# SamsungLabs/Metis

Hardware: AMD Instinct MI355X
Metric: best_plan_iter_time_ms (lower is better)
Workload: dtype bf16; 1 GPU; model=gpt3-2.7b, global_batch=16, seq_len=2048, parallelism=dp1_tp1_pp1, microbatch=16

## Files before the change

metis_amd/ops/hip/attention.hip:

```cpp

#include <torch/extension.h>
#include <c10/hip/HIPStream.h>

#include "attn_host.h"
#include "attn_tile.h"

namespace {

using namespace attn_tile;

constexpr int THREADS = 256;
constexpr int QBLK = 128;
constexpr int RESIDENT = 2;
static_assert(QBLK == ATTN_SEQ_TILE, "check_attn_qkv pins S to this tile");

template <int D>
constexpr int kvblk_for() { return D <= 80 ? 128 : 64; }

template <int D>
using FwdLayout = TileLayout<D, kvblk_for<D>(), THREADS / 64 * 2, RESIDENT>;
static_assert(FwdLayout<64>::bytes == 71680 && FwdLayout<80>::bytes == 79872
              && FwdLayout<96>::bytes == 45056 && FwdLayout<128>::bytes == 53248);

template <int D, bool PACKED>
__global__ __launch_bounds__(THREADS, RESIDENT) void attn_fwd_kernel(
    const bf16* __restrict__ Q,
    const bf16* __restrict__ K,
    const bf16* __restrict__ V,
    bf16* __restrict__ O,
    float* __restrict__ LSE,
    int B, int H, int Hkv, int S,
    float scale) {
    const int lane = threadIdx.x & 63;
    const int wave = threadIdx.x >> 6;
    const int col16 = lane & 15;
    const int k8 = lane >> 4;

    using L = FwdLayout<D>;
    constexpr int KVBLK = kvblk_for<D>();
    constexpr int JSUB = KVBLK / 16;
    constexpr int dchunks = Geom<D>::dchunks;
    constexpr int djtiles = Geom<D>::djtiles;
    constexpr int KSLOT = Geom<D>::KSLOT;
    constexpr int VROW = L::WROW;

    const BlockCoord bc = block_coord<D, PACKED>(S / QBLK, H, Hkv, S);
    const long q_base = bc.q_base;
    const int pitch = bc.qkv_pitch;

    const int rbid[2] = {wave, 7 - wave};
    const int qb = bc.tile * QBLK;

    extern __shared__ __attribute__((aligned(16))) char smem[];
    short* Ks = reinterpret_cast<short*>(smem) + L::a_off;
    short* Vs = reinterpret_cast<short*>(smem) + L::b_off;
    short* Pw = reinterpret_cast<short*>(smem) + L::w_off + wave * 2 * L::w_tile;

    bf16x8 q_frag[2][dchunks];
    #pragma unroll
    for (int rb = 0; rb < 2; ++rb)
        #pragma unroll
        for (int c = 0; c < dchunks; ++c)
            q_frag[rb][c] = frag8<D>(Q + q_base, qb + rbid[rb] * 16 + col16,
                                     c * 32 + k8 * 8, pitch);

    float m_run[2][4], l_run[2][4];
    #pragma unroll
    for (int rb = 0; rb < 2; ++rb)
        #pragma unroll
        for (int r = 0; r < 4; ++r) {
            m_run[rb][r] = -1e30f;
            l_run[rb][r] = 0.f;
        }
    floatx4 o_acc[2][djtiles] = {};

    constexpr Walk WK = PACKED ? Walk::WholeRows : Walk::DChunksInRow;
    constexpr Walk WV = PACKED ? Walk::WholeRows : Walk::RowsInDChunk;
    TileStage<KVBLK, D, THREADS, WK, WV, true,
              PACKED> stage;
    const bf16* Kh = K + bc.kv_base;
    const bf16* Vh = V + bc.kv_base;

    const int kv_end = qb + QBLK;
    stage.issue_loads(Kh, Vh, 0, pitch, pitch);
    for (int kv0 = 0; kv0 < kv_end; kv0 += KVBLK) {
        stage.write_stage(Ks, Vs, Vh, kv0, pitch);
        if (kv0 + KVBLK < kv_end) stage.issue_loads(Kh, Vh, kv0 + KVBLK, pitch,
                                                      pitch);
        __syncthreads();

        bool rb_active[2];
        float p[2][JSUB][4];
        #pragma unroll
        for (int rb = 0; rb < 2; ++rb) {
            const int q0 = qb + rbid[rb] * 16;
            rb_active[rb] = kv0 <= q0 + 15;
            if (!rb_active[rb]) continue;

            __builtin_amdgcn_s_setprio(1);
            #pragma unroll
            for (int j = 0; j < JSUB; ++j) {
                floatx4 s_acc = floatx4{0.f, 0.f, 0.f, 0.f};
                const int kvrow = j * 16 + col16;
                #pragma unroll
                for (int c = 0; c < dchunks; ++c) {
                    const bf16x8 k_frag =
                        lds_frag<D, KSLOT>(Ks, kvrow, c * 32 + k8 * 8);
                    s_acc = __builtin_amdgcn_mfma_f32_16x16x32_bf16(
                        q_frag[rb][c], k_frag, s_acc, 0, 0, 0);
                }
                #pragma unroll
                for (int r = 0; r < 4; ++r) {
                    const int qrow = q0 + k8 * 4 + r;
                    const int kvcol = kv0 + j * 16 + col16;
                    float sv = s_acc[r] * scale;
                    p[rb][j][r] = (kvcol > qrow) ? -1e30f : sv;
                }
            }
            __builtin_amdgcn_s_setprio(0);

            #pragma unroll
            for (int r = 0; r < 4; ++r) {
                float tile_max = -1e30f;
                #pragma unroll
                for (int j = 0; j < JSUB; ++j)
                    tile_max = fmaxf(tile_max, p[rb][j][r]);
                #pragma unroll
                for (int off = 8; off > 0; off >>= 1)
                    tile_max = fmaxf(tile_max, __shfl_xor(tile_max, off, 16));

                const float m_new = fmaxf(m_run[rb][r], tile_max);
                const float alpha = __expf(m_run[rb][r] - m_new);
                float row_sum = 0.f;
                #pragma unroll
                for (int j = 0; j < JSUB; ++j) {
                    p[rb][j][r] = __expf(p[rb][j][r] - m_new);
                    row_sum += p[rb][j][r];
                }
                #pragma unroll
                for (int off = 8; off > 0; off >>= 1)
                    row_sum += __shfl_xor(row_sum, off, 16);

                l_run[rb][r] = l_run[rb][r] * alpha + row_sum;
                m_run[rb][r] = m_new;
                #pragma unroll
                for (int jd = 0; jd < djtiles; ++jd)
                    o_acc[rb][jd][r] *= alpha;
            }

            short* Prb = Pw + rb * 16 * VROW;
            #pragma unroll
            for (int j = 0; j < JSUB; ++j)
                #pragma unroll
                for (int r = 0; r < 4; ++r)
                    Prb[(k8 * 4 + r) * VROW + j * 16 + col16] =
                        float_to_bf16_bits(p[rb][j][r]);
        }

        asm volatile("" ::: "memory");

        #pragma unroll
        for (int rb = 0; rb < 2; ++rb) {
            if (!rb_active[rb]) continue;
            const short* Prb = Pw + rb * 16 * VROW;
            #pragma unroll
            for (int ks = 0; ks < KVBLK / 32; ++ks) {
                bf16x8 p_frag = *reinterpret_cast<const bf16x8*>(
                    Prb + col16 * VROW + ks * 32 + k8 * 8);
                #pragma unroll
                for (int jd = 0; jd < djtiles; ++jd) {
                    const bf16x8 v_frag = tr16_frag<KSLOT>(
                        Vs, ks * 32 + k8 * 8, jd * 16, col16);
                    o_acc[rb][jd] = __builtin_amdgcn_mfma_f32_16x16x32_bf16(
                        p_frag, v_frag, o_acc[rb][jd], 0, 0, 0);
                }
            }
        }
        __syncthreads();
    }

    #pragma unroll
    for (int rb = 0; rb < 2; ++rb) {
        #pragma unroll
        for (int r = 0; r < 4; ++r) {
            const int qrow = qb + rbid[rb] * 16 + k8 * 4 + r;
            const float inv_l = 1.f / l_run[rb][r];
            #pragma unroll
            for (int jd = 0; jd < djtiles; ++jd)
                O[bc.o_base + (long)qrow * bc.o_pitch + jd * 16 + col16] =
                    __float2bfloat16(o_acc[rb][jd][r] * inv_l);
            if (col16 == 0)
                LSE[bc.row_base + qrow] =
                    m_run[rb][r] + __logf(l_run[rb][r]);
        }
    }
}

}

std::vector<torch::Tensor> attn_fwd(
    torch::Tensor q, torch::Tensor k, torch::Tensor v, double scale) {
    const AttnDims a = check_attn_qkv(q, k, v);
    auto qc = q.contiguous(), kc = k.contiguous(), vc = v.contiguous();

    auto o = torch::empty_like(qc);
    auto lse = torch::empty({a.B, a.H, a.S}, q.options().dtype(torch::kFloat32));

    const int grid = (int)(a.B * a.H * (a.S / QBLK));
    auto stream = c10::hip::getCurrentHIPStream().stream();
    dispatch_head_dim(a.D, [&](auto d) {
        constexpr int DD = decltype(d)::value;
        hipLaunchKernelGGL((attn_fwd_kernel<DD, false>), dim3(grid), dim3(THREADS),
            FwdLayout<DD>::bytes, stream,
            bf16_ptr(qc), bf16_ptr(kc), bf16_ptr(vc), bf16_ptr(o),
            lse.data_ptr<float>(),
            (int)a.B, (int)a.H, (int)a.Hkv, (int)a.S, (float)scale);
    });
    HIP_CHECK_LAST();
    return {o, lse};
}

std::vector<torch::Tensor> attn_fwd_packed(
    torch::Tensor qkv, long H, long Hkv, long D, double scale) {
    const AttnDims a = check_attn_packed_qkv(qkv, H, Hkv, D);

    auto o = torch::empty({a.B, a.S, a.H * a.D}, qkv.options());
    auto lse = torch::empty({a.B, a.H, a.S}, qkv.options().dtype(torch::kFloat32));
// ... 16 lines not shown
```

metis_amd/ops/hip/attention_bwd.hip:

```cpp

#include <torch/extension.h>
#include <c10/hip/HIPStream.h>

#include "attn_host.h"
#include "attn_tile.h"

namespace {

using namespace attn_tile;

constexpr int THREADS = 256;
constexpr int RBLK = 128;
constexpr int CTILE = 64;
constexpr int VROW = CTILE + VPAD;
constexpr int RESIDENT = 2;
static_assert(RBLK == ATTN_SEQ_TILE, "check_attn_qkv pins S to this tile");

template <int D>
constexpr int dkv_rows() { return D == 64 ? 128 : 64; }

template <int D>
using DqLayout = TileLayout<D, CTILE, THREADS / 64 * 2, RESIDENT>;
template <int D>
using DkvLayout = TileLayout<D, CTILE, 2 * (dkv_rows<D>() / 16), RESIDENT>;
static_assert(DqLayout<64>::bytes == 36864 && DqLayout<80>::bytes == 40960
              && DqLayout<96>::bytes == 45056 && DqLayout<128>::bytes == 53248);
static_assert(DkvLayout<64>::bytes == 55296 && DkvLayout<80>::bytes == 40960
              && DkvLayout<96>::bytes == 45056 && DkvLayout<128>::bytes == 53248);

template <int D, bool PACKED>
__global__ __launch_bounds__(THREADS, RESIDENT) void attn_bwd_dq_kernel(
    const bf16* __restrict__ Q, const bf16* __restrict__ K,
    const bf16* __restrict__ V, const bf16* __restrict__ dO,
    const float* __restrict__ LSE, const float* __restrict__ Delta,
    bf16* __restrict__ dQ,
    int B, int H, int Hkv, int S, float scale) {
    const int lane = threadIdx.x & 63;
    const int wave = threadIdx.x >> 6;
    const int col16 = lane & 15;
    const int k8 = lane >> 4;

    using L = DqLayout<D>;
    constexpr int dchunks = Geom<D>::dchunks;
    constexpr int djtiles = Geom<D>::djtiles;
    constexpr int KSLOT = Geom<D>::KSLOT;

    const BlockCoord bc = block_coord<D, PACKED>(S / RBLK, H, Hkv, S);
    const long q_base = bc.q_base, row_base = bc.row_base;
    const int pitch = bc.qkv_pitch;

    const int rbid[2] = {wave, 7 - wave};
    const int qb = bc.tile * RBLK;

    extern __shared__ __attribute__((aligned(16))) char smem[];
    short* Ks = reinterpret_cast<short*>(smem) + L::a_off;
    short* Vs = reinterpret_cast<short*>(smem) + L::b_off;
    short* Sw = reinterpret_cast<short*>(smem) + L::w_off + wave * 2 * L::w_tile;

    float lse_r[2][4], delta_r[2][4];
    bf16x8 q_frag[2][dchunks], do_frag[2][dchunks];
    #pragma unroll
    for (int rb = 0; rb < 2; ++rb) {
        const int q0 = qb + rbid[rb] * 16;
        #pragma unroll
        for (int r = 0; r < 4; ++r) {
            lse_r[rb][r] = LSE[row_base + q0 + k8 * 4 + r];
            delta_r[rb][r] = Delta[row_base + q0 + k8 * 4 + r];
        }
        #pragma unroll
        for (int c = 0; c < dchunks; ++c) {
            q_frag[rb][c] = frag8<D>(Q + q_base, q0 + col16, c * 32 + k8 * 8,
                                     pitch);
            do_frag[rb][c] = frag8<D>(dO + bc.o_base, q0 + col16,
                                      c * 32 + k8 * 8, bc.o_pitch);
        }
    }

    floatx4 dq_acc[2][djtiles] = {};

    constexpr Walk WALK = PACKED ? Walk::WholeRows : Walk::RowsInDChunk;
    TileStage<CTILE, D, THREADS, WALK, WALK, false,
              PACKED> stage;
    const bf16* Kh = K + bc.kv_base;
    const bf16* Vh = V + bc.kv_base;

    const int kv_end = qb + RBLK;
    stage.issue_loads(Kh, Vh, 0, pitch, pitch);
    for (int kv0 = 0; kv0 < kv_end; kv0 += CTILE) {
        stage.write_stage(Ks, Vs, Vh, kv0, pitch);
        if (kv0 + CTILE < kv_end)
            stage.issue_loads(Kh, Vh, kv0 + CTILE, pitch, pitch);
        __syncthreads();

        bool rb_active[2];
        #pragma unroll
        for (int rb = 0; rb < 2; ++rb) {
            const int q0 = qb + rbid[rb] * 16;
            rb_active[rb] = kv0 <= q0 + 15;
            if (!rb_active[rb]) continue;

            __builtin_amdgcn_s_setprio(1);
            floatx4 s_acc[4], dp_acc[4];
            #pragma unroll
            for (int j = 0; j < 4; ++j) {
                s_acc[j] = floatx4{0.f, 0.f, 0.f, 0.f};
                dp_acc[j] = floatx4{0.f, 0.f, 0.f, 0.f};
                const int kvrow = j * 16 + col16;
                #pragma unroll
                for (int c = 0; c < dchunks; ++c) {
                    const int d0 = c * 32 + k8 * 8;
                    bf16x8 kf, vf;
                    lds_frag2<D, KSLOT>(Ks, Vs, kvrow, d0, kf, vf);
                    s_acc[j] = __builtin_amdgcn_mfma_f32_16x16x32_bf16(
                        q_frag[rb][c], kf, s_acc[j], 0, 0, 0);
                    dp_acc[j] = __builtin_amdgcn_mfma_f32_16x16x32_bf16(
                        do_frag[rb][c], vf, dp_acc[j], 0, 0, 0);
                }
            }
            __builtin_amdgcn_s_setprio(0);

            short* Srb = Sw + rb * 16 * VROW;
            #pragma unroll
            for (int j = 0; j < 4; ++j)
                #pragma unroll
                for (int r = 0; r < 4; ++r) {
                    const int qrow = q0 + k8 * 4 + r;
                    const int kvcol = kv0 + j * 16 + col16;
                    float p = (kvcol > qrow)
                                  ? 0.f
                                  : __expf(s_acc[j][r] * scale - lse_r[rb][r]);
                    float ds = scale * p * (dp_acc[j][r] - delta_r[rb][r]);
                    Srb[(k8 * 4 + r) * VROW + j * 16 + col16] =
                        float_to_bf16_bits(ds);
                }
        }

        asm volatile("" ::: "memory");

        #pragma unroll
        for (int rb = 0; rb < 2; ++rb) {
            if (!rb_active[rb]) continue;
            const short* Srb = Sw + rb * 16 * VROW;
            #pragma unroll
            for (int ks = 0; ks < 2; ++ks) {
                bf16x8 ds_frag = *reinterpret_cast<const bf16x8*>(
                    Srb + col16 * VROW + ks * 32 + k8 * 8);
                #pragma unroll
                for (int jd = 0; jd < djtiles; ++jd) {
                    bf16x8 kt_frag = tr16_frag<KSLOT>(
                        Ks, ks * 32 + k8 * 8, jd * 16, col16);
                    dq_acc[rb][jd] = __builtin_amdgcn_mfma_f32_16x16x32_bf16(
                        ds_frag, kt_frag, dq_acc[rb][jd], 0, 0, 0);
                }
            }
        }
        __syncthreads();
    }

    #pragma unroll
    for (int rb = 0; rb < 2; ++rb)
        #pragma unroll
        for (int r = 0; r < 4; ++r) {
            const long qrow = qb + rbid[rb] * 16 + k8 * 4 + r;
            #pragma unroll
            for (int jd = 0; jd < djtiles; ++jd)
                dQ[q_base + qrow * pitch + jd * 16 + col16] =
                    __float2bfloat16(dq_acc[rb][jd][r]);
        }
}

template <int D, bool PACKED>
__global__ __launch_bounds__(dkv_rows<D>() / 16 * 64, RESIDENT)
void attn_bwd_dkv_kernel(
    const bf16* __restrict__ Q, const bf16* __restrict__ K,
    const bf16* __restrict__ V, const bf16* __restrict__ dO,
    const float* __restrict__ LSE, const float* __restrict__ Delta,
    bf16* __restrict__ dK,
    bf16* __restrict__ dV,
    int B, int H, int Hkv, int S, float scale) {
    const int lane = threadIdx.x & 63;
    const int wave = threadIdx.x >> 6;
    const int col16 = lane & 15;
    const int k8 = lane >> 4;

    using L = DkvLayout<D>;
    constexpr int dchunks = Geom<D>::dchunks;
    constexpr int djtiles = Geom<D>::djtiles;
    constexpr int KSLOT = Geom<D>::KSLOT;
    constexpr int KVB = dkv_rows<D>();
    constexpr int NW = KVB / 16;

    const BlockCoord bc = block_coord<D, PACKED>(S / KVB, H, Hkv, S);
    const long kv_base = bc.kv_base, row_base = bc.row_base;
    const long out_base = bc.q_base;
    const int pitch = bc.qkv_pitch;

    const int kv0 = bc.tile * KVB + wave * 16;

    extern __shared__ __attribute__((aligned(16))) char smem[];
    short* Qs = reinterpret_cast<short*>(smem) + L::a_off;
    short* dOs = reinterpret_cast<short*>(smem) + L::b_off;
    short* Sw = reinterpret_cast<short*>(smem) + L::w_off + wave * L::w_tile;
    short* Pw = reinterpret_cast<short*>(smem) + L::w_off + (NW + wave) * L::w_tile;

    bf16x8 k_frag[dchunks], v_frag[dchunks];
    #pragma unroll
    for (int c = 0; c < dchunks; ++c) {
        k_frag[c] = frag8<D>(K + kv_base, kv0 + col16, c * 32 + k8 * 8, pitch);
        v_frag[c] = frag8<D>(V + kv_base, kv0 + col16, c * 32 + k8 * 8, pitch);
    }

    floatx4 dk_acc[djtiles] = {}, dv_acc[djtiles] = {};

    constexpr bool STAGE_DO = (D <= 96);
    constexpr Walk WALK = PACKED ? Walk::WholeRows : Walk::RowsInDChunk;
    TileStage<CTILE, D, NW * 64, WALK, WALK, STAGE_DO,
              PACKED> stage;
    const bf16* Qh = Q + bc.q_base;
    const bf16* dOh = dO + bc.o_base;

    const int q_start = bc.tile * KVB;
    stage.issue_loads(Qh, dOh, q_start, pitch, bc.o_pitch);
    for (int q0 = q_start; q0 < S; q0 += CTILE) {
        stage.write_stage(Qs, dOs, dOh, q0, bc.o_pitch);
        if (q0 + CTILE < S)
            stage.issue_loads(Qh, dOh, q0 + CTILE, pitch, bc.o_pitch);
        __syncthreads();

        const bool active = q0 + CTILE - 1 >= kv0;
        if (active) {
            __builtin_amdgcn_s_setprio(1);
            floatx4 st_acc[4], dpt_acc[4];
            #pragma unroll
            for (int j = 0; j < 4; ++j) {
                st_acc[j] = floatx4{0.f, 0.f, 0.f, 0.f};
                dpt_acc[j] = floatx4{0.f, 0.f, 0.f, 0.f};
                const int qrow = j * 16 + col16;
                #pragma unroll
                for (int c = 0; c < dchunks; ++c) {
                    const int d0 = c * 32 + k8 * 8;
                    bf16x8 qf, dof;
                    lds_frag2<D, KSLOT>(Qs, dOs, qrow, d0, qf, dof);
                    st_acc[j] = __builtin_amdgcn_mfma_f32_16x16x32_bf16(
                        k_frag[c], qf, st_acc[j], 0, 0, 0);
                    dpt_acc[j] = __builtin_amdgcn_mfma_f32_16x16x32_bf16(
                        v_frag[c], dof, dpt_acc[j], 0, 0, 0);
                }
            }
            __builtin_amdgcn_s_setprio(0);

            #pragma unroll
            for (int j = 0; j < 4; ++j)
                #pragma unroll
                for (int r = 0; r < 4; ++r) {
                    const int kvrow = kv0 + k8 * 4 + r;
                    const int qcol = q0 + j * 16 + col16;
                    float p = (qcol < kvrow)
                                  ? 0.f
                                  : __expf(st_acc[j][r] * scale
                                           - LSE[row_base + qcol]);
                    float ds = scale * p
                               * (dpt_acc[j][r] - Delta[row_base + qcol]);
                    Sw[(k8 * 4 + r) * VROW + j * 16 + col16] =
                        float_to_bf16_bits(ds);
                    Pw[(k8 * 4 + r) * VROW + j * 16 + col16] =
                        float_to_bf16_bits(p);
                }

            asm volatile("" ::: "memory");

            #pragma unroll
            for (int ks = 0; ks < 2; ++ks) {
                bf16x8 dst_frag = *reinterpret_cast<const bf16x8*>(
                    Sw + col16 * VROW + ks * 32 + k8 * 8);
                bf16x8 pt_frag = *reinterpret_cast<const bf16x8*>(
                    Pw + col16 * VROW + ks * 32 + k8 * 8);
                #pragma unroll
                for (int jd = 0; jd < djtiles; ++jd) {
                    bf16x8 qt_frag = tr16_frag<KSLOT>(
                        Qs, ks * 32 + k8 * 8, jd * 16, col16);
                    dk_acc[jd] = __builtin_amdgcn_mfma_f32_16x16x32_bf16(
                        dst_frag, qt_frag, dk_acc[jd], 0, 0, 0);
                    bf16x8 dot_frag = tr16_frag<KSLOT>(
                        dOs, ks * 32 + k8 * 8, jd * 16, col16);
                    dv_acc[jd] = __builtin_amdgcn_mfma_f32_16x16x32_bf16(
                        pt_frag, dot_frag, dv_acc[jd], 0, 0, 0);
                }
            }
        }
        __syncthreads();
    }

    #pragma unroll
    for (int r = 0; r < 4; ++r) {
        const long kvrow = kv0 + k8 * 4 + r;
        #pragma unroll
        for (int jd = 0; jd < djtiles; ++jd) {
            dK[out_base + kvrow * pitch + jd * 16 + col16] =
                __float2bfloat16(dk_acc[jd][r]);
            dV[out_base + kvrow * pitch + jd * 16 + col16] =
                __float2bfloat16(dv_acc[jd][r]);
        }
    }
}

constexpr int DELTA_THREADS = 256;
constexpr int DELTA_U = 4;

template <bool PACKED>
__global__ void __launch_bounds__(DELTA_THREADS) attn_bwd_delta_kernel(
    const bf16x8* __restrict__ o,
    const bf16x8* __restrict__ d_o,
    float* __restrict__ delta,
    long rows,
    int dv,
    int H, int S) {
    const int sub = threadIdx.x & 15;
    const bool live = sub < dv;
    const int ci = live ? sub : dv - 1;
    const long rows_per_block = DELTA_THREADS / 16 * DELTA_U;
// ... 66 lines not shown
    const long rows = B * S * H;
    auto delta = torch::empty({B, H, S}, o.options().dtype(torch::kFloat32));
    const long rows_per_block = DELTA_THREADS / 16 * DELTA_U;
    const long grid = (rows + rows_per_block - 1) / rows_per_block;
    hipLaunchKernelGGL(attn_bwd_delta_kernel<true>, dim3((unsigned)grid),
        dim3(DELTA_THREADS), 0, c10::hip::getCurrentHIPStream().stream(),
        reinterpret_cast<const bf16x8*>(o.data_ptr()),
        reinterpret_cast<const bf16x8*>(d_o.data_ptr()),
        delta.data_ptr<float>(), rows, (int)(D / 8), (int)H, (int)S);
    HIP_CHECK_LAST();
    return delta;
}

std::vector<torch::Tensor> attn_bwd(
    torch::Tensor q, torch::Tensor k, torch::Tensor v,
    torch::Tensor d_o, torch::Tensor lse, torch::Tensor delta,
    double scale) {
    const AttnDims a = check_attn_qkv(q, k, v);
    TORCH_CHECK(d_o.is_cuda() && d_o.dtype() == torch::kBFloat16,
                "d_o must be CUDA bf16");
    TORCH_CHECK(lse.is_cuda() && lse.dtype() == torch::kFloat32
                && delta.is_cuda() && delta.dtype() == torch::kFloat32,
                "lse and delta must be CUDA fp32");
    for (const torch::Tensor* t : {&d_o, &lse, &delta})
        TORCH_CHECK(t->get_device() == q.get_device(),
                    "all attn_bwd arguments must be on the same device");
    TORCH_CHECK(d_o.sizes() == q.sizes(), "d_o must be [B, H, S, D] like q");
    TORCH_CHECK(lse.dim() == 3 && lse.size(0) == a.B && lse.size(1) == a.H
                && lse.size(2) == a.S, "lse must be [B, H, S]");
    TORCH_CHECK(delta.sizes() == lse.sizes(), "delta must be [B, H, S]");
    auto qc = q.contiguous(), kc = k.contiguous(), vc = v.contiguous();
    auto doc = d_o.contiguous();
    auto lsec = lse.contiguous(), dc = delta.contiguous();

    auto dq = torch::empty_like(qc);
    auto dk = torch::empty({a.B, a.H, a.S, a.D}, q.options());
    auto dv = torch::empty({a.B, a.H, a.S, a.D}, q.options());

    auto stream = c10::hip::getCurrentHIPStream().stream();
    dispatch_head_dim(a.D, [&](auto d) {
        constexpr int DD = decltype(d)::value;
        const int grid_dq = (int)(a.B * a.H * (a.S / RBLK));
        hipLaunchKernelGGL((attn_bwd_dq_kernel<DD, false>), dim3(grid_dq),
            dim3(THREADS), DqLayout<DD>::bytes, stream,
            bf16_ptr(qc), bf16_ptr(kc), bf16_ptr(vc), bf16_ptr(doc),
            lsec.data_ptr<float>(), dc.data_ptr<float>(), bf16_ptr(dq),
            (int)a.B, (int)a.H, (int)a.Hkv, (int)a.S, (float)scale);
        constexpr int KVB = dkv_rows<DD>();
        const int grid_dkv = (int)(a.B * a.H * (a.S / KVB));
        hipLaunchKernelGGL((attn_bwd_dkv_kernel<DD, false>), dim3(grid_dkv),
            dim3(KVB / 16 * 64), DkvLayout<DD>::bytes, stream,
            bf16_ptr(qc), bf16_ptr(kc), bf16_ptr(vc), bf16_ptr(doc),
            lsec.data_ptr<float>(), dc.data_ptr<float>(),
            bf16_ptr(dk), bf16_ptr(dv),
            (int)a.B, (int)a.H, (int)a.Hkv, (int)a.S, (float)scale);
    });
    HIP_CHECK_LAST();
    return {dq, dk, dv};
}

torch::Tensor attn_bwd_packed(
    torch::Tensor qkv, torch::Tensor d_o, torch::Tensor lse, torch::Tensor delta,
    long H, long Hkv, long D, double scale) {
    const AttnDims a = check_attn_packed_qkv(qkv, H, Hkv, D);
    check_attn_packed_out(d_o, "d_o", qkv, a.B, a.S, a.H, a.D);
    check_attn_rows(lse, "lse", qkv, a.B, a.H, a.S);
// ... 29 lines not shown
```

metis_amd/ops/hip/attn_host.h:

```cpp
#pragma once

#include <torch/extension.h>

#include <type_traits>

#include "common.h"

struct AttnDims { long B, H, Hkv, S, D; };

constexpr int ATTN_SEQ_TILE = 128;

inline AttnDims check_attn_qkv(const torch::Tensor& q, const torch::Tensor& k,
                               const torch::Tensor& v, bool decode = false) {
    TORCH_CHECK(q.is_cuda() && q.dtype() == torch::kBFloat16, "q must be CUDA bf16");
    TORCH_CHECK(q.dim() == 4, "q must be [B, H, S, D] (S = 1 for decode)");
    TORCH_CHECK(k.is_cuda() && k.dtype() == torch::kBFloat16
                && v.is_cuda() && v.dtype() == torch::kBFloat16,
                "k and v must be CUDA bf16");
    TORCH_CHECK(k.get_device() == q.get_device()
                && v.get_device() == q.get_device(),
                "q, k and v must be on the same device");
    TORCH_CHECK(k.dim() == 4 && v.dim() == 4 && k.sizes() == v.sizes(),
                "k and v must both be [B, Hkv, S, D]");
    const AttnDims d{q.size(0), q.size(1), k.size(1), k.size(2), q.size(3)};
// ... 19 lines not shown
                name, " must be CUDA bf16");
    TORCH_CHECK(t.dim() == 3, name, " must be [B, S, heads * D]");
    TORCH_CHECK(t.is_contiguous(), name, " must be contiguous");
    TORCH_CHECK(reinterpret_cast<uintptr_t>(t.data_ptr()) % 16 == 0,
                name, " must be 16-byte aligned");
}

inline AttnDims check_attn_packed_qkv(const torch::Tensor& qkv, long H, long Hkv,
                                      long D) {
    check_attn_packed_operand(qkv, "qkv");
    check_head_dim(D);
    TORCH_CHECK(H > 0 && H == Hkv,
                "packed attention needs H == Hkv > 0, got H=", H, " Hkv=", Hkv);
    TORCH_CHECK(qkv.size(2) == (H + 2 * Hkv) * D,
                "qkv width must be (H + 2 * Hkv) * D");
    const AttnDims d{qkv.size(0), H, Hkv, qkv.size(1), D};
    TORCH_CHECK(d.B > 0 && d.S > 0 && d.S % ATTN_SEQ_TILE == 0,
                "sequence length must be a positive multiple of 128");
    TORCH_CHECK(d.B * d.H * d.S < (1L << 31) && qkv.size(2) < (1L << 24),
                "B * H * S must fit an int and the row pitch be below 2^24");
    return d;
}

inline void check_attn_packed_out(const torch::Tensor& t, const char* name,
                                  const torch::Tensor& like, long B, long S,
                                  long H, long D) {
    check_attn_packed_operand(t, name);
    TORCH_CHECK(t.get_device() == like.get_device(),
                name, " must be on the same device as the other arguments");
    TORCH_CHECK(t.size(0) == B && t.size(1) == S && t.size(2) == H * D,
                name, " must be [B, S, H * D]");
}

inline void check_attn_rows(const torch::Tensor& t, const char* name,
                            const torch::Tensor& like, long B, long H, long S) {
    TORCH_CHECK(t.is_cuda() && t.dtype() == torch::kFloat32,
                name, " must be CUDA fp32");
    TORCH_CHECK(t.get_device() == like.get_device(),
                name, " must be on the same device as the other arguments");
    TORCH_CHECK(t.dim() == 3 && t.size(0) == B && t.size(1) == H
                && t.size(2) == S && t.is_contiguous(),
                name, " must be a contiguous [B, H, S]");
}

template <class F>
void dispatch_head_dim(long D, F&& f) {
    check_head_dim(D);
    switch (D) {
        case 64: f(std::integral_constant<int, 64>{}); break;
        case 80: f(std::integral_constant<int, 80>{}); break;
        case 96: f(std::integral_constant<int, 96>{}); break;
        default: f(std::integral_constant<int, 128>{}); break;
    }
}

inline bf16* bf16_ptr(const torch::Tensor& t) {
    return reinterpret_cast<bf16*>(t.data_ptr());
}
```

metis_amd/ops/hip/attn_tile.h:

```cpp
#pragma once

#include "common.h"

namespace attn_tile {

typedef short short4v __attribute__((ext_vector_type(4)));

constexpr int VPAD = 8;
constexpr int LDS_PER_CU = 160 * 1024;

template <int D>
struct Geom {
    static constexpr int dchunks = (D + 31) / 32;
    static constexpr int djtiles = D / 16;
    static constexpr int KSLOT = D / 8 + 1;
    static constexpr int tile(int rows) { return rows * KSLOT * 8; }
};

template <int D, int ROWS, int WTILES, int RESIDENT>
struct TileLayout {
    static constexpr int WROW = ROWS + VPAD;
    static constexpr int a_off = 0;
    static constexpr int b_off = Geom<D>::tile(ROWS);
    static constexpr int w_off = 2 * Geom<D>::tile(ROWS);
    static constexpr int w_tile = 16 * WROW;
    static constexpr int bytes = (w_off + WTILES * w_tile) * 2;
    static_assert(b_off % 8 == 0 && w_off % 8 == 0 && w_tile % 8 == 0);
    static_assert(bytes * RESIDENT <= LDS_PER_CU, "resident blocks must fit one CU");
};

template <int D>
__device__ __forceinline__ bf16x8 frag8(const bf16* base, long row, int d0,
                                        int pitch) {
    if (d0 < D)
        return *reinterpret_cast<const bf16x8*>(base + row * pitch + d0);
    return bf16x8{0, 0, 0, 0, 0, 0, 0, 0};
}

template <int D, int KSLOT>
__device__ __forceinline__ bf16x8 lds_frag(const short* img, int row, int d0) {
    if (d0 < D)
        return *reinterpret_cast<const bf16x8*>(img + row * KSLOT * 8 + d0);
    return bf16x8{0, 0, 0, 0, 0, 0, 0, 0};
}

template <int D, int KSLOT>
__device__ __forceinline__ void lds_frag2(const short* img_a, const short* img_b,
                                          int row, int d0, bf16x8& a, bf16x8& b) {
    a = b = bf16x8{0, 0, 0, 0, 0, 0, 0, 0};
    if (d0 < D) {
        a = *reinterpret_cast<const bf16x8*>(img_a + row * KSLOT * 8 + d0);
        b = *reinterpret_cast<const bf16x8*>(img_b + row * KSLOT * 8 + d0);
    }
}

template <int KSLOT>
__device__ __forceinline__ bf16x8 tr16_frag(
    const short* img, int row0, int col0, int p4) {
    bf16x8 out;
    #pragma unroll
    for (int r = 0; r < 2; ++r) {
        const int row = row0 + 4 * r + (p4 >> 2);
        const int col = col0 + (p4 & 3) * 4;
        short4v t = __builtin_amdgcn_ds_read_tr16_b64_v4i16(
            (__attribute__((address_space(3))) short4v*)(
                img + row * KSLOT * 8 + col));
        out[r * 4 + 0] = t[0];
        out[r * 4 + 1] = t[1];
        out[r * 4 + 2] = t[2];
        out[r * 4 + 3] = t[3];
    }
    return out;
}

struct BlockCoord {
    int tile;
    long q_base, kv_base;
    long o_base;
    long row_base;
    int qkv_pitch;
    int o_pitch;
};

template <int D, bool PACKED>
__device__ __forceinline__ BlockCoord block_coord(int tiles, int H, int Hkv, int S) {
    const int head = (blockIdx.x / tiles) % H;
    const int batch = blockIdx.x / tiles / H;
    BlockCoord c;
    c.tile = blockIdx.x % tiles;
    c.row_base = ((long)batch * H + head) * S;
    if constexpr (PACKED) {
        const int HT = H + 2 * Hkv;
        c.qkv_pitch = HT * D;
        c.o_pitch = H * D;
        c.q_base = c.kv_base = ((long)batch * S * HT + head) * D;
        c.o_base = ((long)batch * S * H + head) * D;
    } else {
        const int kv_head = head / (H / Hkv);
        c.qkv_pitch = c.o_pitch = D;
        c.q_base = c.o_base = c.row_base * D;
        c.kv_base = (((long)batch * Hkv + kv_head) * S) * D;
    }
    return c;
}

enum class Walk { DChunksInRow, RowsInDChunk, WholeRows };
// ... 88 lines not shown
```

Baseline: 784.6 ms.

## Keep softmax probabilities in registers by transposing MFMA operands in attention kernels

Forward and backward attention kernels swap MFMA operand order so the S/P accumulator layout matches the B-operand fragment layout. P and dS then pack directly into bf16 fragments in registers instead of taking a round trip through per-wave LDS scratch, and the scratch region is removed from the LDS layouts. Row-block pairs now share K/V fragment loads across two MFMAs. Launch bounds change per head dim, and the output store is vectorised. This cuts LDS traffic and footprint and may raise occupancy, at the cost of more register pressure and a reordered transposed-read pattern.

```diff
diff --git a/metis_amd/ops/hip/attention.hip b/metis_amd/ops/hip/attention.hip
--- a/metis_amd/ops/hip/attention.hip
+++ b/metis_amd/ops/hip/attention.hip
@@ -17,10 +17,13 @@
 template <int D>
 constexpr int kvblk_for() { return D <= 80 ? 128 : 64; }
 
+template <int D, bool PACKED>
+constexpr bool pair_rows() { return D == 64 || D == 96 || (D == 80 && PACKED); }
+
 template <int D>
-using FwdLayout = TileLayout<D, kvblk_for<D>(), THREADS / 64 * 2, RESIDENT>;
-static_assert(FwdLayout<64>::bytes == 71680 && FwdLayout<80>::bytes == 79872
-              && FwdLayout<96>::bytes == 45056 && FwdLayout<128>::bytes == 53248);
+using FwdLayout = TileLayout<D, kvblk_for<D>(), 0, RESIDENT>;
+static_assert(FwdLayout<64>::bytes == 36864 && FwdLayout<80>::bytes == 45056
+              && FwdLayout<96>::bytes == 26624 && FwdLayout<128>::bytes == 34816);
 
 template <int D, bool PACKED>
 __global__ __launch_bounds__(THREADS, RESIDENT) void attn_fwd_kernel(
@@ -32,7 +35,7 @@
     int B, int H, int Hkv, int S,
     float scale) {
     const int lane = threadIdx.x & 63;
-    const int wave = threadIdx.x >> 6;
+    const int wave = __builtin_amdgcn_readfirstlane(threadIdx.x >> 6);
     const int col16 = lane & 15;
     const int k8 = lane >> 4;
 
@@ -42,7 +45,6 @@
     constexpr int dchunks = Geom<D>::dchunks;
     constexpr int djtiles = Geom<D>::djtiles;
     constexpr int KSLOT = Geom<D>::KSLOT;
-    constexpr int VROW = L::WROW;
 
     const BlockCoord bc = block_coord<D, PACKED>(S / QBLK, H, Hkv, S);
     const long q_base = bc.q_base;
@@ -54,7 +56,6 @@
     extern __shared__ __attribute__((aligned(16))) char smem[];
     short* Ks = reinterpret_cast<short*>(smem) + L::a_off;
     short* Vs = reinterpret_cast<short*>(smem) + L::b_off;
-    short* Pw = reinterpret_cast<short*>(smem) + L::w_off + wave * 2 * L::w_tile;
 
     bf16x8 q_frag[2][dchunks];
     #pragma unroll
@@ -64,14 +65,7 @@
             q_frag[rb][c] = frag8<D>(Q + q_base, qb + rbid[rb] * 16 + col16,
                                      c * 32 + k8 * 8, pitch);
 
-    float m_run[2][4], l_run[2][4];
-    #pragma unroll
-    for (int rb = 0; rb < 2; ++rb)
-        #pragma unroll
-        for (int r = 0; r < 4; ++r) {
-            m_run[rb][r] = -1e30f;
-            l_run[rb][r] = 0.f;
-        }
+    float m_run[2] = {-1e30f, -1e30f}, l_run[2] = {0.f, 0.f};
     floatx4 o_acc[2][djtiles] = {};
 
     constexpr Walk WK = PACKED ? Walk::WholeRows : Walk::DChunksInRow;
@@ -80,6 +74,86 @@
               PACKED> stage;
     const bf16* Kh = K + bc.kv_base;
     const bf16* Vh = V + bc.kv_base;
+
+    auto tile_body = [&](auto rb_lo, auto rb_hi, int kv0) {
+        constexpr int RB0 = decltype(rb_lo)::value, RB1 = decltype(rb_hi)::value;
+
+        float p[2][JSUB][4];
+        __builtin_amdgcn_s_setprio(1);
+        #pragma unroll
+        for (int j = 0; j < JSUB; ++j) {
+            floatx4 s_acc[2] = {};
+            #pragma unroll
+            for (int c = 0; c < dchunks; ++c) {
+                const bf16x8 k_frag =
+                    lds_frag<D, KSLOT>(Ks, j * 16 + col16, c * 32 + k8 * 8);
+                #pragma unroll
+                for (int rb = RB0; rb < RB1; ++rb)
+                    s_acc[rb] = __builtin_amdgcn_mfma_f32_16x16x32_bf16(
+                        k_frag, q_frag[rb][c], s_acc[rb], 0, 0, 0);
+            }
+            #pragma unroll
+            for (int rb = RB0; rb < RB1; ++rb) {
+                const int qrow = qb + rbid[rb] * 16 + col16;
+                #pragma unroll
+                for (int r = 0; r < 4; ++r) {
+                    const int kvrow = kv0 + j * 16 + k8 * 4 + r;
+                    p[rb][j][r] = (kvrow > qrow) ? -1e30f : s_acc[rb][r] * scale;
+                }
+            }
+        }
+        __builtin_amdgcn_s_setprio(0);
+        __builtin_amdgcn_sched_barrier(0);
+
+        AccFrag p_frag[2][KVBLK / 32];
+        #pragma unroll
+        for (int rb = RB0; rb < RB1; ++rb) {
+            float tile_max = -1e30f;
+            #pragma unroll
+            for (int j = 0; j < JSUB; ++j)
+                #pragma unroll
+                for (int r = 0; r < 4; ++r)
+                    tile_max = fmaxf(tile_max, p[rb][j][r]);
+            tile_max = fmaxf(tile_max, __shfl_xor(tile_max, 16, WAVE_SIZE));
+            tile_max = fmaxf(tile_max, __shfl_xor(tile_max, 32, WAVE_SIZE));
+
+            const float m_new = fmaxf(m_run[rb], tile_max);
+            const float alpha = __expf(m_run[rb] - m_new);
+            float row_sum = 0.f;
+            #pragma unroll
+            for (int j = 0; j < JSUB; ++j) {
+                floatx4 e;
+                #pragma unroll
+                for (int r = 0; r < 4; ++r) {
+                    e[r] = __expf(p[rb][j][r] - m_new);
+                    row_sum += e[r];
+                }
+                p_frag[rb][j >> 1].set_half(j & 1, e);
+            }
+            row_sum += __shfl_xor(row_sum, 16, WAVE_SIZE);
+            row_sum += __shfl_xor(row_sum, 32, WAVE_SIZE);
+
+            l_run[rb] = l_run[rb] * alpha + row_sum;
+            m_run[rb] = m_new;
+            #pragma unroll
+            for (int jd = 0; jd < djtiles; ++jd)
+                o_acc[rb][jd] *= alpha;
+        }
+
+        __builtin_amdgcn_sched_barrier(0);
+        #pragma unroll
+        for (int ks = 0; ks < KVBLK / 32; ++ks) {
+            #pragma unroll
+            for (int jd = 0; jd < djtiles; ++jd) {
+                const bf16x8 vt_frag = tr16_frag_acc<KSLOT>(
+                    Vs, ks * 32, k8, jd * 16, col16);
+                #pragma unroll
+                for (int rb = RB0; rb < RB1; ++rb)
+                    o_acc[rb][jd] = __builtin_amdgcn_mfma_f32_16x16x32_bf16(
+                        vt_frag, p_frag[rb][ks].frag(), o_acc[rb][jd], 0, 0, 0);
+            }
+        }
+    };
 
     const int kv_end = qb + QBLK;
     stage.issue_loads(Kh, Vh, 0, pitch, pitch);
@@ -89,110 +163,35 @@
                                                       pitch);
         __syncthreads();
 
-        bool rb_active[2];
-        float p[2][JSUB][4];
-        #pragma unroll
-        for (int rb = 0; rb < 2; ++rb) {
-            const int q0 = qb + rbid[rb] * 16;
-            rb_active[rb] = kv0 <= q0 + 15;
-            if (!rb_active[rb]) continue;
-
-            __builtin_amdgcn_s_setprio(1);
-            #pragma unroll
-            for (int j = 0; j < JSUB; ++j) {
-                floatx4 s_acc = floatx4{0.f, 0.f, 0.f, 0.f};
-                const int kvrow = j * 16 + col16;
-                #pragma unroll
-                for (int c = 0; c < dchunks; ++c) {
-                    const bf16x8 k_frag =
-                        lds_frag<D, KSLOT>(Ks, kvrow, c * 32 + k8 * 8);
-                    s_acc = __builtin_amdgcn_mfma_f32_16x16x32_bf16(
-                        q_frag[rb][c], k_frag, s_acc, 0, 0, 0);
-                }
-                #pragma unroll
-                for (int r = 0; r < 4; ++r) {
-                    const int qrow = q0 + k8 * 4 + r;
-                    const int kvcol = kv0 + j * 16 + col16;
-                    float sv = s_acc[r] * scale;
-                    p[rb][j][r] = (kvcol > qrow) ? -1e30f : sv;
-                }
-            }
-            __builtin_amdgcn_s_setprio(0);
-
-            #pragma unroll
-            for (int r = 0; r < 4; ++r) {
-                float tile_max = -1e30f;
-                #pragma unroll
-                for (int j = 0; j < JSUB; ++j)
-                    tile_max = fmaxf(tile_max, p[rb][j][r]);
-                #pragma unroll
-                for (int off = 8; off > 0; off >>= 1)
-                    tile_max = fmaxf(tile_max, __shfl_xor(tile_max, off, 16));
-
-                const float m_new = fmaxf(m_run[rb][r], tile_max);
-                const float alpha = __expf(m_run[rb][r] - m_new);
-                float row_sum = 0.f;
-                #pragma unroll
-                for (int j = 0; j < JSUB; ++j) {
-                    p[rb][j][r] = __expf(p[rb][j][r] - m_new);
-                    row_sum += p[rb][j][r];
-                }
-                #pragma unroll
-                for (int off = 8; off > 0; off >>= 1)
-                    row_sum += __shfl_xor(row_sum, off, 16);
-
-                l_run[rb][r] = l_run[rb][r] * alpha + row_sum;
-                m_run[rb][r] = m_new;
-                #pragma unroll
-                for (int jd = 0; jd < djtiles; ++jd)
-                    o_acc[rb][jd][r] *= alpha;
-            }
-
-            short* Prb = Pw + rb * 16 * VROW;
-            #pragma unroll
-            for (int j = 0; j < JSUB; ++j)
-                #pragma unroll
-                for (int r = 0; r < 4; ++r)
-                    Prb[(k8 * 4 + r) * VROW + j * 16 + col16] =
-                        float_to_bf16_bits(p[rb][j][r]);
-        }
-
-        asm volatile("" ::: "memory");
-
-        #pragma unroll
-        for (int rb = 0; rb < 2; ++rb) {
-            if (!rb_active[rb]) continue;
-            const short* Prb = Pw + rb * 16 * VROW;
-            #pragma unroll
-            for (int ks = 0; ks < KVBLK / 32; ++ks) {
-                bf16x8 p_frag = *reinterpret_cast<const bf16x8*>(
-                    Prb + col16 * VROW + ks * 32 + k8 * 8);
-                #pragma unroll
-                for (int jd = 0; jd < djtiles; ++jd) {
-                    const bf16x8 v_frag = tr16_frag<KSLOT>(
-                        Vs, ks * 32 + k8 * 8, jd * 16, col16);
-                    o_acc[rb][jd] = __builtin_amdgcn_mfma_f32_16x16x32_bf16(
-                        p_frag, v_frag, o_acc[rb][jd], 0, 0, 0);
-                }
-            }
+        const bool early_live = KVBLK == QBLK || kv0 <= qb + rbid[0] * 16 + 15;
+        constexpr std::integral_constant<int, 0> i0;
+        constexpr std::integral_constant<int, 1> i1;
+        constexpr std::integral_constant<int, 2> i2;
+        if constexpr (pair_rows<D, PACKED>()) {
+            if (early_live) tile_body(i0, i2, kv0);
+            else tile_body(i1, i2, kv0);
+        } else {
+            if (early_live) tile_body(i0, i1, kv0);
+            tile_body(i1, i2, kv0);
         }
         __syncthreads();
     }
 
     #pragma unroll
     for (int rb = 0; rb < 2; ++rb) {
-        #pragma unroll
-        for (int r = 0; r < 4; ++r) {
-            const int qrow = qb + rbid[rb] * 16 + k8 * 4 + r;
-            const float inv_l = 1.f / l_run[rb][r];
-            #pragma unroll
-            for (int jd = 0; jd < djtiles; ++jd)
-                O[bc.o_base + (long)qrow * bc.o_pitch + jd * 16 + col16] =
-                    __float2bfloat16(o_acc[rb][jd][r] * inv_l);
-            if (col16 == 0)
-                LSE[bc.row_base + qrow] =
-                    m_run[rb][r] + __logf(l_run[rb][r]);
-        }
+        const int qrow = qb + rbid[rb] * 16 + col16;
+        const float inv_l = 1.f / l_run[rb];
+        #pragma unroll
+        for (int jd = 0; jd < djtiles; ++jd) {
+            const floatx4 o = o_acc[rb][jd] * inv_l;
+            uint2 packed;
+            packed.x = pack_bf16x2(o[0], o[1]);
+            packed.y = pack_bf16x2(o[2], o[3]);
+            *reinterpret_cast<uint2*>(
+                O + bc.o_base + (long)qrow * bc.o_pitch + jd * 16 + k8 * 4) = packed;
+        }
+        if (k8 == 0)
+            LSE[bc.row_base + qrow] = m_run[rb] + __logf(l_run[rb]);
     }
 }
 
diff --git a/metis_amd/ops/hip/attention_bwd.hip b/metis_amd/ops/hip/attention_bwd.hip
--- a/metis_amd/ops/hip/attention_bwd.hip
+++ b/metis_amd/ops/hip/attention_bwd.hip
@@ -12,7 +12,6 @@
 constexpr int THREADS = 256;
 constexpr int RBLK = 128;
 constexpr int CTILE = 64;
-constexpr int VROW = CTILE + VPAD;
 constexpr int RESIDENT = 2;
 static_assert(RBLK == ATTN_SEQ_TILE, "check_attn_qkv pins S to this tile");
 
@@ -20,23 +19,29 @@
 constexpr int dkv_rows() { return D == 64 ? 128 : 64; }
 
 template <int D>
-using DqLayout = TileLayout<D, CTILE, THREADS / 64 * 2, RESIDENT>;
-template <int D>
-using DkvLayout = TileLayout<D, CTILE, 2 * (dkv_rows<D>() / 16), RESIDENT>;
-static_assert(DqLayout<64>::bytes == 36864 && DqLayout<80>::bytes == 40960
-              && DqLayout<96>::bytes == 45056 && DqLayout<128>::bytes == 53248);
-static_assert(DkvLayout<64>::bytes == 55296 && DkvLayout<80>::bytes == 40960
-              && DkvLayout<96>::bytes == 45056 && DkvLayout<128>::bytes == 53248);
+constexpr int dq_waves() { return D == 64 ? 3 : 2; }
+template <int D>
+constexpr int dkv_waves() { return D == 64 ? 4 : D == 80 ? 3 : 2; }
+
+template <int D>
+constexpr bool dq_pair_rows() { return D == 96; }
+
+template <int D>
+using DqLayout = TileLayout<D, CTILE, 0, RESIDENT>;
+template <int D>
+using DkvLayout = TileLayout<D, CTILE, 0, RESIDENT>;
+static_assert(DqLayout<64>::bytes == 18432 && DqLayout<80>::bytes == 22528
+              && DqLayout<96>::bytes == 26624 && DqLayout<128>::bytes == 34816);
 
 template <int D, bool PACKED>
-__global__ __launch_bounds__(THREADS, RESIDENT) void attn_bwd_dq_kernel(
+__global__ __launch_bounds__(THREADS, dq_waves<D>()) void attn_bwd_dq_kernel(
     const bf16* __restrict__ Q, const bf16* __restrict__ K,
     const bf16* __restrict__ V, const bf16* __restrict__ dO,
     const float* __restrict__ LSE, const float* __restrict__ Delta,
     bf16* __restrict__ dQ,
     int B, int H, int Hkv, int S, float scale) {
     const int lane = threadIdx.x & 63;
-    const int wave = threadIdx.x >> 6;
+    const int wave = __builtin_amdgcn_readfirstlane(threadIdx.x >> 6);
     const int col16 = lane & 15;
     const int k8 = lane >> 4;
 
@@ -55,18 +60,14 @@
     extern __shared__ __attribute__((aligned(16))) char smem[];
     short* Ks = reinterpret_cast<short*>(smem) + L::a_off;
     short* Vs = reinterpret_cast<short*>(smem) + L::b_off;
-    short* Sw = reinterpret_cast<short*>(smem) + L::w_off + wave * 2 * L::w_tile;
-
-    float lse_r[2][4], delta_r[2][4];
+
+    float lse_c[2], delta_c[2];
     bf16x8 q_frag[2][dchunks], do_frag[2][dchunks];
     #pragma unroll
     for (int rb = 0; rb < 2; ++rb) {
         const int q0 = qb + rbid[rb] * 16;
-        #pragma unroll
-        for (int r = 0; r < 4; ++r) {
-            lse_r[rb][r] = LSE[row_base + q0 + k8 * 4 + r];
-            delta_r[rb][r] = Delta[row_base + q0 + k8 * 4 + r];
-        }
+        lse_c[rb] = LSE[row_base + q0 + col16];
+        delta_c[rb] = Delta[row_base + q0 + col16];
         #pragma unroll
         for (int c = 0; c < dchunks; ++c) {
             q_frag[rb][c] = frag8<D>(Q + q_base, q0 + col16, c * 32 + k8 * 8,
@@ -83,6 +84,60 @@
               PACKED> stage;
     const bf16* Kh = K + bc.kv_base;
     const bf16* Vh = V + bc.kv_base;
+
+    auto tile_body = [&](auto rb_lo, auto rb_hi, int kv0) {
+        constexpr int RB0 = decltype(rb_lo)::value, RB1 = decltype(rb_hi)::value;
+
+        AccFrag ds_frag[2][CTILE / 32];
+        __builtin_amdgcn_s_setprio(1);
+        #pragma unroll
+        for (int j = 0; j < CTILE / 16; ++j) {
+            floatx4 st_acc[2] = {}, dpt_acc[2] = {};
+            #pragma unroll
+            for (int c = 0; c < dchunks; ++c) {
+                bf16x8 kf, vf;
+                lds_frag2<D, KSLOT>(Ks, Vs, j * 16 + col16, c * 32 + k8 * 8,
+                                    kf, vf);
+                #pragma unroll
+                for (int rb = RB0; rb < RB1; ++rb) {
+                    st_acc[rb] = __builtin_amdgcn_mfma_f32_16x16x32_bf16(
+                        kf, q_frag[rb][c], st_acc[rb], 0, 0, 0);
+                    dpt_acc[rb] = __builtin_amdgcn_mfma_f32_16x16x32_bf16(
+                        vf, do_frag[rb][c], dpt_acc[rb], 0, 0, 0);
+                }
+            }
+            #pragma unroll
+            for (int rb = RB0; rb < RB1; ++rb) {
+                const int qrow = qb + rbid[rb] * 16 + col16;
+                floatx4 ds;
+                #pragma unroll
+                for (int r = 0; r < 4; ++r) {
+                    const int kvrow = kv0 + j * 16 + k8 * 4 + r;
+                    const float p =
+                        (kvrow > qrow)
+                            ? 0.f
+                            : __expf(st_acc[rb][r] * scale - lse_c[rb]);
+                    ds[r] = scale * p * (dpt_acc[rb][r] - delta_c[rb]);
+                }
+                ds_frag[rb][j >> 1].set_half(j & 1, ds);
+            }
+        }
+        __builtin_amdgcn_s_setprio(0);
+        __builtin_amdgcn_sched_barrier(0);
+
+        #pragma unroll
+        for (int ks = 0; ks < CTILE / 32; ++ks) {
+            #pragma unroll
+            for (int jd = 0; jd < djtiles; ++jd) {
+                const bf16x8 kt_frag = tr16_frag_acc<KSLOT>(
+                    Ks, ks * 32, k8, jd * 16, col16);
+                #pragma unroll
+                for (int rb = RB0; rb < RB1; ++rb)
+                    dq_acc[rb][jd] = __builtin_amdgcn_mfma_f32_16x16x32_bf16(
+                        ds_frag[rb][ks].frag(), kt_frag, dq_acc[rb][jd], 0, 0, 0);
+            }
+        }
+    };
 
     const int kv_end = qb + RBLK;
     stage.issue_loads(Kh, Vh, 0, pitch, pitch);
@@ -92,67 +147,16 @@
             stage.issue_loads(Kh, Vh, kv0 + CTILE, pitch, pitch);
         __syncthreads();
 
-        bool rb_active[2];
-        #pragma unroll
-        for (int rb = 0; rb < 2; ++rb) {
-            const int q0 = qb + rbid[rb] * 16;
-            rb_active[rb] = kv0 <= q0 + 15;
-            if (!rb_active[rb]) continue;
-
-            __builtin_amdgcn_s_setprio(1);
-            floatx4 s_acc[4], dp_acc[4];
-            #pragma unroll
-            for (int j = 0; j < 4; ++j) {
-                s_acc[j] = floatx4{0.f, 0.f, 0.f, 0.f};
-                dp_acc[j] = floatx4{0.f, 0.f, 0.f, 0.f};
-                const int kvrow = j * 16 + col16;
-                #pragma unroll
-                for (int c = 0; c < dchunks; ++c) {
-                    const int d0 = c * 32 + k8 * 8;
-                    bf16x8 kf, vf;
-                    lds_frag2<D, KSLOT>(Ks, Vs, kvrow, d0, kf, vf);
-                    s_acc[j] = __builtin_amdgcn_mfma_f32_16x16x32_bf16(
-                        q_frag[rb][c], kf, s_acc[j], 0, 0, 0);
-                    dp_acc[j] = __builtin_amdgcn_mfma_f32_16x16x32_bf16(
-                        do_frag[rb][c], vf, dp_acc[j], 0, 0, 0);
-                }
-            }
-            __builtin_amdgcn_s_setprio(0);
-
-            short* Srb = Sw + rb * 16 * VROW;
-            #pragma unroll
-            for (int j = 0; j < 4; ++j)
-                #pragma unroll
-                for (int r = 0; r < 4; ++r) {
-                    const int qrow = q0 + k8 * 4 + r;
-                    const int kvcol = kv0 + j * 16 + col16;
-                    float p = (kvcol > qrow)
-                                  ? 0.f
-                                  : __expf(s_acc[j][r] * scale - lse_r[rb][r]);
-                    float ds = scale * p * (dp_acc[j][r] - delta_r[rb][r]);
-                    Srb[(k8 * 4 + r) * VROW + j * 16 + col16] =
-                        float_to_bf16_bits(ds);
-                }
-        }
-
-        asm volatile("" ::: "memory");
-
-        #pragma unroll
-        for (int rb = 0; rb < 2; ++rb) {
-            if (!rb_active[rb]) continue;
-            const short* Srb = Sw + rb * 16 * VROW;
-            #pragma unroll
-            for (int ks = 0; ks < 2; ++ks) {
-                bf16x8 ds_frag = *reinterpret_cast<const bf16x8*>(
-                    Srb + col16 * VROW + ks * 32 + k8 * 8);
-                #pragma unroll
-                for (int jd = 0; jd < djtiles; ++jd) {
-                    bf16x8 kt_frag = tr16_frag<KSLOT>(
-                        Ks, ks * 32 + k8 * 8, jd * 16, col16);
-                    dq_acc[rb][jd] = __builtin_amdgcn_mfma_f32_16x16x32_bf16(
-                        ds_frag, kt_frag, dq_acc[rb][jd], 0, 0, 0);
-                }
-            }
+        const bool early_live = kv0 <= qb + rbid[0] * 16 + 15;
+        constexpr std::integral_constant<int, 0> i0;
+        constexpr std::integral_constant<int, 1> i1;
+        constexpr std::integral_constant<int, 2> i2;
+        if constexpr (dq_pair_rows<D>()) {
+            if (early_live) tile_body(i0, i2, kv0);
+            else tile_body(i1, i2, kv0);
+        } else {
+            if (early_live) tile_body(i0, i1, kv0);
+            tile_body(i1, i2, kv0);
         }
         __syncthreads();
     }
@@ -170,7 +174,7 @@
 }
 
 template <int D, bool PACKED>
-__global__ __launch_bounds__(dkv_rows<D>() / 16 * 64, RESIDENT)
+__global__ __launch_bounds__(dkv_rows<D>() / 16 * 64, dkv_waves<D>())
 void attn_bwd_dkv_kernel(
     const bf16* __restrict__ Q, const bf16* __restrict__ K,
     const bf16* __restrict__ V, const bf16* __restrict__ dO,
@@ -179,7 +183,7 @@
     bf16* __restrict__ dV,
     int B, int H, int Hkv, int S, float scale) {
     const int lane = threadIdx.x & 63;
-    const int wave = threadIdx.x >> 6;
+    const int wave = __builtin_amdgcn_readfirstlane(threadIdx.x >> 6);
     const int col16 = lane & 15;
     const int k8 = lane >> 4;
 
@@ -200,8 +204,6 @@
     extern __shared__ __attribute__((aligned(16))) char smem[];
     short* Qs = reinterpret_cast<short*>(smem) + L::a_off;
     short* dOs = reinterpret_cast<short*>(smem) + L::b_off;
-    short* Sw = reinterpret_cast<short*>(smem) + L::w_off + wave * L::w_tile;
-    short* Pw = reinterpret_cast<short*>(smem) + L::w_off + (NW + wave) * L::w_tile;
 
     bf16x8 k_frag[dchunks], v_frag[dchunks];
     #pragma unroll
@@ -222,70 +224,77 @@
     const int q_start = bc.tile * KVB;
     stage.issue_loads(Qh, dOh, q_start, pitch, bc.o_pitch);
     for (int q0 = q_start; q0 < S; q0 += CTILE) {
+        const bool active = q0 + CTILE - 1 >= kv0;
+        float4 lse4[2], delta4[2];
+        auto load_rows = [&](int ks) {
+            #pragma unroll
+            for (int jj = 0; jj < 2; ++jj) {
+                const long q = row_base + q0 + ks * 32 + jj * 16 + k8 * 4;
+                lse4[jj] = *reinterpret_cast<const float4*>(LSE + q);
+                delta4[jj] = *reinterpret_cast<const float4*>(Delta + q);
+            }
+        };
+        if (active) load_rows(0);
+
         stage.write_stage(Qs, dOs, dOh, q0, bc.o_pitch);
         if (q0 + CTILE < S)
             stage.issue_loads(Qh, dOh, q0 + CTILE, pitch, bc.o_pitch);
         __syncthreads();
 
-        const bool active = q0 + CTILE - 1 >= kv0;
         if (active) {
-            __builtin_amdgcn_s_setprio(1);
-            floatx4 st_acc[4], dpt_acc[4];
-            #pragma unroll
-            for (int j = 0; j < 4; ++j) {
-                st_acc[j] = floatx4{0.f, 0.f, 0.f, 0.f};
-                dpt_acc[j] = floatx4{0.f, 0.f, 0.f, 0.f};
-                const int qrow = j * 16 + col16;
+            #pragma unroll
+            for (int ks = 0; ks < CTILE / 32; ++ks) {
+                AccFrag p_frag, ds_frag;
+                __builtin_amdgcn_s_setprio(1);
                 #pragma unroll
-                for (int c = 0; c < dchunks; ++c) {
-                    const int d0 = c * 32 + k8 * 8;
-                    bf16x8 qf, dof;
-                    lds_frag2<D, KSLOT>(Qs, dOs, qrow, d0, qf, dof);
-                    st_acc[j] = __builtin_amdgcn_mfma_f32_16x16x32_bf16(
-                        k_frag[c], qf, st_acc[j], 0, 0, 0);
-                    dpt_acc[j] = __builtin_amdgcn_mfma_f32_16x16x32_bf16(
-                        v_frag[c], dof, dpt_acc[j], 0, 0, 0);
+                for (int jj = 0; jj < 2; ++jj) {
+                    const int j = ks * 2 + jj;
+                    floatx4 s_acc = {}, dp_acc = {};
+                    #pragma unroll
+                    for (int c = 0; c < dchunks; ++c) {
+                        bf16x8 qf, dof;
+                        lds_frag2<D, KSLOT>(Qs, dOs, j * 16 + col16,
+                                            c * 32 + k8 * 8, qf, dof);
+                        s_acc = __builtin_amdgcn_mfma_f32_16x16x32_bf16(
+                            qf, k_frag[c], s_acc, 0, 0, 0);
+                        dp_acc = __builtin_amdgcn_mfma_f32_16x16x32_bf16(
+                            dof, v_frag[c], dp_acc, 0, 0, 0);
+                    }
+                    const float lse_r[4] = {lse4[jj].x, lse4[jj].y, lse4[jj].z,
+                                            lse4[jj].w};
+                    const float delta_r[4] = {delta4[jj].x, delta4[jj].y,
+                                              delta4[jj].z, delta4[jj].w};
+                    floatx4 p, ds;
+                    #pragma unroll
+                    for (int r = 0; r < 4; ++r) {
+                        const int qrow = q0 + j * 16 + k8 * 4 + r;
+                        const int kvrow = kv0 + col16;
+                        p[r] = (qrow < kvrow)
+                                   ? 0.f
+                                   : __expf(s_acc[r] * scale - lse_r[r]);
+                        ds[r] = scale * p[r] * (dp_acc[r] - delta_r[r]);
+                    }
+                    p_frag.set_half(jj, p);
+                    ds_frag.set_half(jj, ds);
                 }
-            }
-            __builtin_amdgcn_s_setprio(0);
-
-            #pragma unroll
-            for (int j = 0; j < 4; ++j)
-                #pragma unroll
-                for (int r = 0; r < 4; ++r) {
-                    const int kvrow = kv0 + k8 * 4 + r;
-                    const int qcol = q0 + j * 16 + col16;
-                    float p = (qcol < kvrow)
-                                  ? 0.f
-                                  : __expf(st_acc[j][r] * scale
-                                           - LSE[row_base + qcol]);
-                    float ds = scale * p
-                               * (dpt_acc[j][r] - Delta[row_base + qcol]);
-                    Sw[(k8 * 4 + r) * VROW + j * 16 + col16] =
-                        float_to_bf16_bits(ds);
-                    Pw[(k8 * 4 + r) * VROW + j * 16 + col16] =
-                        float_to_bf16_bits(p);
-                }
-
-            asm volatile("" ::: "memory");
-
-            #pragma unroll
-            for (int ks = 0; ks < 2; ++ks) {
-                bf16x8 dst_frag = *reinterpret_cast<const bf16x8*>(
-                    Sw + col16 * VROW + ks * 32 + k8 * 8);
-                bf16x8 pt_frag = *reinterpret_cast<const bf16x8*>(
-                    Pw + col16 * VROW + ks * 32 + k8 * 8);
+                __builtin_amdgcn_s_setprio(0);
+                __builtin_amdgcn_sched_barrier(0);
+                if (ks + 1 < CTILE / 32) load_rows(ks + 1);
+
+                const bf16x8 dst_frag = ds_frag.frag();
+                const bf16x8 pt_frag = p_frag.frag();
                 #pragma unroll
                 for (int jd = 0; jd < djtiles; ++jd) {
-                    bf16x8 qt_frag = tr16_frag<KSLOT>(
-                        Qs, ks * 32 + k8 * 8, jd * 16, col16);
+                    bf16x8 qt_frag = tr16_frag_acc<KSLOT>(
+                        Qs, ks * 32, k8, jd * 16, col16);
                     dk_acc[jd] = __builtin_amdgcn_mfma_f32_16x16x32_bf16(
                         dst_frag, qt_frag, dk_acc[jd], 0, 0, 0);
-                    bf16x8 dot_frag = tr16_frag<KSLOT>(
-                        dOs, ks * 32 + k8 * 8, jd * 16, col16);
+                    bf16x8 dot_frag = tr16_frag_acc<KSLOT>(
+                        dOs, ks * 32, k8, jd * 16, col16);
                     dv_acc[jd] = __builtin_amdgcn_mfma_f32_16x16x32_bf16(
                         pt_frag, dot_frag, dv_acc[jd], 0, 0, 0);
                 }
+                __builtin_amdgcn_sched_barrier(0);
             }
         }
         __syncthreads();
@@ -418,6 +427,8 @@
     auto qc = q.contiguous(), kc = k.contiguous(), vc = v.contiguous();
     auto doc = d_o.contiguous();
     auto lsec = lse.contiguous(), dc = delta.contiguous();
+    check_attn_rows_aligned(lsec, "lse");
+    check_attn_rows_aligned(dc, "delta");
 
     auto dq = torch::empty_like(qc);
     auto dk = torch::empty({a.B, a.H, a.S, a.D}, q.options());
diff --git a/metis_amd/ops/hip/attn_host.h b/metis_amd/ops/hip/attn_host.h
--- a/metis_amd/ops/hip/attn_host.h
+++ b/metis_amd/ops/hip/attn_host.h
@@ -75,6 +75,11 @@
                 name, " must be [B, S, H * D]");
 }
 
+inline void check_attn_rows_aligned(const torch::Tensor& t, const char* name) {
+    TORCH_CHECK(reinterpret_cast<uintptr_t>(t.data_ptr()) % 16 == 0,
+                name, " must be 16-byte aligned");
+}
+
 inline void check_attn_rows(const torch::Tensor& t, const char* name,
                             const torch::Tensor& like, long B, long H, long S) {
     TORCH_CHECK(t.is_cuda() && t.dtype() == torch::kFloat32,
@@ -84,6 +89,7 @@
     TORCH_CHECK(t.dim() == 3 && t.size(0) == B && t.size(1) == H
                 && t.size(2) == S && t.is_contiguous(),
                 name, " must be a contiguous [B, H, S]");
+    check_attn_rows_aligned(t, name);
 }
 
 template <class F>
diff --git a/metis_amd/ops/hip/attn_tile.h b/metis_amd/ops/hip/attn_tile.h
--- a/metis_amd/ops/hip/attn_tile.h
+++ b/metis_amd/ops/hip/attn_tile.h
@@ -55,12 +55,12 @@
 }
 
 template <int KSLOT>
-__device__ __forceinline__ bf16x8 tr16_frag(
-    const short* img, int row0, int col0, int p4) {
+__device__ __forceinline__ bf16x8 tr16_rows(
+    const short* img, int row_lo, int row_hi, int col0, int p4) {
     bf16x8 out;
     #pragma unroll
     for (int r = 0; r < 2; ++r) {
-        const int row = row0 + 4 * r + (p4 >> 2);
+        const int row = (r ? row_hi : row_lo) + (p4 >> 2);
         const int col = col0 + (p4 & 3) * 4;
         short4v t = __builtin_amdgcn_ds_read_tr16_b64_v4i16(
             (__attribute__((address_space(3))) short4v*)(
@@ -72,6 +72,37 @@
     }
     return out;
 }
+
+template <int KSLOT>
+__device__ __forceinline__ bf16x8 tr16_frag(
+    const short* img, int row0, int col0, int p4) {
+    return tr16_rows<KSLOT>(img, row0, row0 + 4, col0, p4);
+}
+
+template <int KSLOT>
+__device__ __forceinline__ bf16x8 tr16_frag_acc(
+    const short* img, int chunk, int g, int col0, int p4) {
+    return tr16_rows<KSLOT>(img, chunk + 4 * g, chunk + 16 + 4 * g, col0, p4);
+}
+
+__device__ __forceinline__ unsigned pack_bf16x2(float lo, float hi) {
+    typedef float floatx2 __attribute__((ext_vector_type(2)));
+    typedef __bf16 bf16x2v __attribute__((ext_vector_type(2)));
+    return __builtin_bit_cast(
+        unsigned, __builtin_convertvector(floatx2{lo, hi}, bf16x2v));
+}
+
+struct AccFrag {
+    unsigned w[4];
+    __device__ __forceinline__ void set_half(int hi, floatx4 x) {
+        w[2 * hi + 0] = pack_bf16x2(x[0], x[1]);
+        w[2 * hi + 1] = pack_bf16x2(x[2], x[3]);
+    }
+    __device__ __forceinline__ bf16x8 frag() const {
+        typedef unsigned uintx4 __attribute__((ext_vector_type(4)));
+        return __builtin_bit_cast(bf16x8, uintx4{w[0], w[1], w[2], w[3]});
+    }
+};
 
 struct BlockCoord {
     int tile;
```

After: 693.4 ms, median of 6. 11.6% less time.
